# SmartBFT-Go/consensus

Hardware: NVIDIA H100
Metric: ECDSA-P256 verifies/sec at batch=64K (higher is better)
Workload: dtype u32 limbs (integer)

## Files before the change

### consensus_b200/csrc/hostsim.h

```cpp
#pragma once
#if defined(SBV_HOSTSIM) && !defined(__CUDACC__)
#include <stdint.h>
#include <string.h>

#include <condition_variable>
#include <map>
#include <mutex>

#define __device__
#define __host__
#define __global__
#define __forceinline__ inline
#define __noinline__
#define __restrict__
#define __shared__
#define __constant__ static const
#define __launch_bounds__(...)

struct hostsim_dim3 { unsigned x = 1, y = 1, z = 1; };
extern thread_local hostsim_dim3 threadIdx, blockIdx, blockDim, gridDim;
struct uint4 { uint32_t x, y, z, w; };
struct uint2 { uint32_t x, y; };
static inline uint4 make_uint4(uint32_t x, uint32_t y, uint32_t z, uint32_t w) { return uint4{x, y, z, w}; }

template <class T> static inline T __ldg(const T *p) { return *p; }
static inline uint32_t __byte_perm(uint32_t x, uint32_t y, uint32_t s) {
    const uint64_t v = ((uint64_t)y << 32) | x;
    uint32_t r = 0;
    for (int i = 0; i < 4; i++) {
        const uint32_t sel = (s >> (4 * i)) & 0xf;
        uint32_t byte = (uint32_t)(v >> (8 * (sel & 7))) & 0xff;
        if (sel & 8) byte = (byte & 0x80) ? 0xff : 0;
        r |= byte << (8 * i);
    }
    return r;
}
static inline uint32_t __funnelshift_r(uint32_t lo, uint32_t hi, uint32_t sh) {
    return (uint32_t)((((uint64_t)hi << 32) | lo) >> (sh & 31));
}
static inline uint32_t __funnelshift_l(uint32_t lo, uint32_t hi, uint32_t sh) {
    return (uint32_t)(((((uint64_t)hi << 32) | lo) << (sh & 31)) >> 32);
}
static inline int __ffs(int x) { return x ? __builtin_ctz((unsigned)x) + 1 : 0; }
static inline int __clz(int x) { return x ? __builtin_clz((unsigned)x) : 32; }
static inline int __popc(unsigned x) { return __builtin_popcount(x); }
static inline uint32_t __umulhi(uint32_t a, uint32_t b) { return (uint32_t)(((uint64_t)a * b) >> 32); }
static inline void __syncthreads() {}
static inline void __syncwarp(unsigned = 0xffffffffu) {}
static inline void __threadfence() {}
struct hostsim_warp {
    std::mutex m;
    std::condition_variable cv;
    struct Slot { unsigned arrived = 0, gen = 0; uint32_t in[32] = {}, out[32] = {}; };
    std::map<unsigned, Slot> slots;
};
extern thread_local hostsim_warp *hostsim_ctx;
static inline void hostsim_exchange(unsigned mask, uint32_t v, uint32_t (&all)[32]) {
    hostsim_warp *w = hostsim_ctx;
    std::unique_lock<std::mutex> lk(w->m);
    hostsim_warp::Slot &s = w->slots[mask];
    s.in[threadIdx.x & 31] = v;
    if (++s.arrived == (unsigned)__builtin_popcount(mask)) {
        memcpy(s.out, s.in, sizeof s.in);
        s.arrived = 0;
        s.gen++;
        w->cv.notify_all();
    } else {
        const unsigned g = s.gen;
        w->cv.wait(lk, [&] { return s.gen != g; });
    }
    memcpy(all, s.out, sizeof s.out);
}
static inline unsigned __ballot_sync(unsigned mask, int p) {
    if (!hostsim_ctx) return p ? 1u : 0u;
    uint32_t all[32];
    hostsim_exchange(mask, p ? 1u : 0u, all);
    unsigned r = 0;
    for (int i = 0; i < 32; i++) if (((mask >> i) & 1) && all[i]) r |= 1u << i;
    return r;
}
static inline unsigned __activemask() { return 1u; }
static inline unsigned __match_any_sync(unsigned mask, uint32_t v) {
    if (!hostsim_ctx) return 1u << (threadIdx.x & 31);
    uint32_t all[32];
    hostsim_exchange(mask, v, all);
    unsigned r = 0;
    for (int i = 0; i < 32; i++) if (((mask >> i) & 1) && all[i] == v) r |= 1u << i;
    return r;
}
template <class T> static inline T __shfl_sync(unsigned mask, T v, int src) {
    static_assert(sizeof(T) == 4, "32-bit shuffles only");
    if (!hostsim_ctx) return v;
    uint32_t u, all[32];
    memcpy(&u, &v, 4);
    hostsim_exchange(mask, u, all);
    T r;
    memcpy(&r, &all[src & 31], 4);
    return r;
}
template <class T> static inline T __shfl_down_sync(unsigned mask, T v, int delta) {
    if (!hostsim_ctx) return v;
    const int src = (int)(threadIdx.x & 31) + delta;
    const T r = __shfl_sync(mask, v, src > 31 ? (int)(threadIdx.x & 31) : src);
    return src > 31 ? v : r;
}
template <class T> static inline T atomicAdd(T *p, T v) { T o = *p; *p = o + v; return o; }
template <class T> static inline T atomicCAS(T *p, T cmp, T v) { T o = *p; if (o == cmp) *p = v; return o; }
template <class T> static inline T atomicMax(T *p, T v) { T o = *p; if (v > o) *p = v; return o; }
template <class T> static inline T atomicOr(T *p, T v) { T o = *p; *p = o | v; return o; }
typedef int cudaError_t;
typedef void *cudaStream_t;
#endif
```

### consensus_b200/csrc/inst_common.cuh

```cuda
#pragma once
#include "key_cache.cuh"
#include "keygroup.cuh"
#include "ops.h"

namespace sbv {

template <class C> struct Cfg;
template <> struct Cfg<P256> {
    static constexpr int COZ_MINB = 6, GPART_MINB = 6, KT_MINB = 6, COMB_MINB = 6;
    static constexpr bool KT_INL = true, COMB_INL = true;
};
template <> struct Cfg<P384> {
    static constexpr int COZ_MINB = 4, GPART_MINB = 3, KT_MINB = 4;
    static constexpr bool KT_INL = false;
};

template <class C>
cudaError_t op_gtable_init(uint32_t *gtab, cudaStream_t st) {
    const size_t entries = (size_t)C::GWINS << C::GW;
    k_gtable_init<C><<<(unsigned)((entries + 127) / 128), 128, 0, st>>>(gtab);
    return cudaGetLastError();
}

template <class C>
cudaError_t op_prep(uint32_t n, const uint8_t *r, const uint8_t *s, const uint8_t *dig, uint32_t dlen, uint32_t *uw, uint8_t *flags,
                    cudaStream_t st) {
    return launch_prep<C, 8>(n, r, s, dig, dlen, uw, flags, st);
}

template <class C>
cudaError_t op_group(uint32_t n, const uint8_t *qx, const uint8_t *qy, uint32_t seed, uint32_t hmask, uint32_t *htab, uint32_t *rep,
                     uint32_t *kcnt, uint32_t threshold, uint32_t max_keys, int32_t *keyid, uint32_t *keylist, uint32_t *counters,
                     cudaStream_t st) {
    const unsigned blocks = (n + 255) / 256;
    k_kg_insert<<<blocks, 256, 0, st>>>(n, KgXY<C>{qx, qy}, seed, hmask, htab, rep, kcnt);
    k_kg_assign<<<blocks, 256, 0, st>>>(n, rep, kcnt, threshold, max_keys, keyid, keylist, counters);
    return cudaGetLastError();
}

inline cudaError_t op_route(uint32_t n, const uint32_t *rep, const int32_t *keyid, int32_t *item_kid, uint32_t *klist, uint32_t *glist,
                            uint32_t *counters, cudaStream_t st) {
    k_kg_route<<<(n + 255) / 256, 256, 0, st>>>(n, rep, keyid, item_kid, klist, glist, counters);
    return cudaGetLastError();
}

template <class C>
cudaError_t op_gpart(uint32_t n, const uint32_t *uw, const uint32_t *gtab, uint32_t *gacc, cudaStream_t st) {
    constexpr int BLOCK = 64;
    k_gpart<C, BLOCK, Cfg<C>::GPART_MINB><<<(n + BLOCK - 1) / BLOCK, BLOCK, 0, st>>>(n, uw, reinterpret_cast<const uint4 *>(gtab), gacc);
    return cudaGetLastError();
}

template <class C>
cudaError_t op_coz(uint32_t n, const uint8_t *qx, const uint8_t *qy, const uint8_t *r, const uint32_t *uw, const uint8_t *flags,
                   const uint32_t *gtab, uint32_t *tscr, uint8_t *ok, const uint32_t *list, const uint32_t *count, cudaStream_t st) {
    constexpr int BLOCK = 64;
    const size_t smem = (size_t)7 * 2 * C::N * 4 * BLOCK;
    k_verify_coz<C, BLOCK, Cfg<C>::COZ_MINB><<<(n + BLOCK - 1) / BLOCK, BLOCK, smem, st>>>(
        n, qx, qy, r, uw, flags, reinterpret_cast<const uint4 *>(gtab), tscr, ok, list, count);
    return cudaGetLastError();
}

template <class C, int W>
cudaError_t op_kt_build(const uint32_t *nkeys_ptr, uint32_t cap, const uint32_t *keylist, const uint8_t *qx, const uint8_t *qy,
                        uint32_t *bases, uint32_t *hs, uint32_t *ztop, uint32_t *pref, uint32_t *ktab, uint8_t *keyflags, cudaStream_t st) {
    using KT = KeyTab<32 * C::N, W>;
    const unsigned kb = (cap + 63) / 64;
    const unsigned wb = (unsigned)(((size_t)cap * KT::NWIN + 63) / 64);
    k_kt_bases4<C, KT><<<(unsigned)(((size_t)cap * 4 + 127) / 128), 128, 0, st>>>(nkeys_ptr, cap, keylist, qx, qy, bases, keyflags);
    k_kt_fill<C, W><<<wb, 64, 0, st>>>(nkeys_ptr, cap, bases, keyflags, hs, ztop, ktab);
    k_kt_inv<C, KT><<<kb, 64, 0, st>>>(nkeys_ptr, cap, keyflags, ztop, pref);
    k_kt_final<C, KT><<<wb, 64, 0, st>>>(nkeys_ptr, cap, bases, keyflags, hs, ztop, ktab);
    return cudaGetLastError();
}

template <class C, int W>
cudaError_t op_kt_verify_grouped(uint32_t n, const int32_t *kidmap, const uint8_t *keyflags, const uint8_t *r, const uint32_t *uw, const uint8_t *flags,
                                 const uint32_t *gtab, const uint32_t *ktab, uint8_t *ok, const uint32_t *list, const uint32_t *count,
                                 const uint32_t *gacc, cudaStream_t st) {
    constexpr int BLOCK = 64;
    k_verify_kt<C, W, BLOCK, Cfg<C>::KT_MINB, false, Cfg<C>::KT_INL><<<(n + BLOCK - 1) / BLOCK, BLOCK, 0, st>>>(
        n, nullptr, kidmap, 0, keyflags, r, uw, flags, reinterpret_cast<const uint4 *>(gtab), reinterpret_cast<const uint4 *>(ktab), ok, list, count,
        gacc);
    return cudaGetLastError();
}

template <class C, int W>
cudaError_t op_kt_verify_registered(uint32_t n, const uint32_t *slot, const int32_t *slot2local, uint32_t n_slots, const uint8_t *keyflags,
                                    const uint8_t *r, const uint32_t *uw, const uint8_t *flags, const uint32_t *gtab, const uint32_t *ktab,
                                    uint8_t *ok, int warp, cudaStream_t st) {
    constexpr int BLOCK = 64;
    const uint4 *g4 = reinterpret_cast<const uint4 *>(gtab), *k4 = reinterpret_cast<const uint4 *>(ktab);
    if (warp)
        k_verify_kt_warp<C, W><<<(unsigned)(((size_t)n * 32 + 127) / 128), 128, 0, st>>>(n, slot, slot2local, n_slots, keyflags, r, uw, flags, g4, k4, ok);
    else
        k_verify_kt<C, W, BLOCK, Cfg<C>::KT_MINB, true, Cfg<C>::KT_INL><<<(n + BLOCK - 1) / BLOCK, BLOCK, 0, st>>>(
            n, slot, slot2local, n_slots, keyflags, r, uw, flags, g4, k4, ok, nullptr, nullptr, nullptr);
    return cudaGetLastError();
}

template <class C>
cudaError_t op_comb_build(const uint32_t *nkeys_ptr, uint32_t cap, const uint32_t *keylist, const uint8_t *qx, const uint8_t *qy,
                          uint32_t *bases, uint32_t *hs, uint32_t *ztop, uint32_t *pref, uint32_t *ktab, uint8_t *keyflags, cudaStream_t st) {
    using CT = CombTab<C>;
    const unsigned kb = (cap + 63) / 64;
    const unsigned cb = (unsigned)(((size_t)cap * CT::NCHAIN + 63) / 64);
    constexpr bool INL = Cfg<C>::COMB_INL;
    k_kt_bases2<C, CT, INL><<<(unsigned)(((size_t)cap * 2 + 127) / 128), 128, 0, st>>>(nkeys_ptr, cap, keylist, qx, qy, bases, keyflags);
    k_comb_affine<C><<<kb, 64, 0, st>>>(nkeys_ptr, cap, keyflags, bases, pref);
    k_comb_fill<C, INL><<<cb, 64, 0, st>>>(nkeys_ptr, cap, bases, keyflags, hs, ztop, ktab);
    k_kt_inv<C, CT><<<kb, 64, 0, st>>>(nkeys_ptr, cap, keyflags, ztop, pref);
    k_kt_final<C, CT, INL><<<cb, 64, 0, st>>>(nkeys_ptr, cap, bases, keyflags, hs, ztop, ktab);
    return cudaGetLastError();
}

template <class C>
cudaError_t op_comb_verify(uint32_t n, const int32_t *kidmap, const uint8_t *keyflags, const uint8_t *r, const uint32_t *uw, const uint8_t *flags,
                           const uint32_t * , const uint32_t *ktab, uint8_t *ok, const uint32_t *list,
                           const uint32_t *count, const uint32_t *gacc, cudaStream_t st) {
    constexpr int BLOCK = 64;
    k_verify_comb<C, BLOCK, Cfg<C>::COMB_MINB, Cfg<C>::COMB_INL><<<(n + BLOCK - 1) / BLOCK, BLOCK, 0, st>>>(
        n, kidmap, keyflags, r, uw, flags, reinterpret_cast<const uint4 *>(ktab), ok, list, count, gacc);
    return cudaGetLastError();
}

template <class C>
cudaError_t op_kc_lookup(const uint32_t *nkeys_ptr, uint32_t kcap, const uint32_t *keylist, const uint8_t *qx, const uint8_t *qy, KcMap c, uint32_t tw4,
                         int32_t *keyid, uint32_t *lk, uint8_t *keyflags, uint32_t *ktab, cudaStream_t st) {
    k_kc_lookup<<<(unsigned)(((size_t)kcap * 32 + 127) / 128), 128, 0, st>>>(nkeys_ptr, kcap, keylist, KcXY<C>{qx, qy}, c, tw4, keyid, lk, keyflags,
                                                                            reinterpret_cast<uint4 *>(ktab));
    return cudaGetLastError();
}

template <class C>
cudaError_t op_kc_insert(uint32_t kcap, const uint32_t *lk, const uint8_t *qx, const uint8_t *qy, KcMap c, uint32_t tw4, const uint8_t *keyflags,
                         const uint32_t *ktab, cudaStream_t st) {
    k_kc_insert<<<(unsigned)(((size_t)kcap * 32 + 127) / 128), 128, 0, st>>>(kcap, lk, KcXY<C>{qx, qy}, c, tw4, keyflags,
                                                                            reinterpret_cast<const uint4 *>(ktab));
    return cudaGetLastError();
}

template <class C, class KT>
constexpr KtGeom kt_geom() {
    using KS = KtSizes<C, KT>;
    return KtGeom{KS::bases_words(1), KS::hs_words(1), KS::ztop_words(1), KS::ktab_words(1)};
}

}
```

### consensus_b200/csrc/keygroup.cuh

```cuda
#pragma once
#include "kernels.cuh"

namespace sbv {

constexpr uint32_t KG_EMPTY = 0xffffffffu;

SBV_DEV uint32_t kg_mix(uint32_t h, uint32_t w) {
    h = (h ^ w) * 0x9E3779B1u;
    h ^= h >> 15;
    return h * 0x85EBCA77u;
}
template <class C>
SBV_DEV uint32_t kg_hash(const uint8_t *__restrict__ qx_be, const uint8_t *__restrict__ qy_be, uint32_t i, uint32_t seed) {
    const uint32_t *x = reinterpret_cast<const uint32_t *>(qx_be + (size_t)i * C::BYTES);
    const uint32_t *y = reinterpret_cast<const uint32_t *>(qy_be + (size_t)i * C::BYTES);
    uint32_t h = seed;
#pragma unroll
    for (int k = 0; k < C::N; k++) {
        h = kg_mix(h, __ldg(x + k));
        h = kg_mix(h, __ldg(y + k));
    }
    return h ^ (h >> 16);
}
template <class C>
SBV_DEV bool kg_same_key(const uint8_t *__restrict__ qx_be, const uint8_t *__restrict__ qy_be, uint32_t i, uint32_t j) {
    const uint32_t *xi = reinterpret_cast<const uint32_t *>(qx_be + (size_t)i * C::BYTES);
    const uint32_t *xj = reinterpret_cast<const uint32_t *>(qx_be + (size_t)j * C::BYTES);
    const uint32_t *yi = reinterpret_cast<const uint32_t *>(qy_be + (size_t)i * C::BYTES);
    const uint32_t *yj = reinterpret_cast<const uint32_t *>(qy_be + (size_t)j * C::BYTES);
    uint32_t diff = 0;
#pragma unroll
    for (int k = 0; k < C::N; k++) diff |= (__ldg(xi + k) ^ __ldg(xj + k)) | (__ldg(yi + k) ^ __ldg(yj + k));
    return diff == 0;
}

template <class C>
struct KgXY {
    const uint8_t *qx_be, *qy_be;
    SBV_DEV uint32_t hash(uint32_t i, uint32_t seed) const { return kg_hash<C>(qx_be, qy_be, i, seed); }
    SBV_DEV bool same(uint32_t i, uint32_t j) const { return kg_same_key<C>(qx_be, qy_be, i, j); }
};
struct KgKey32 {
    const uint8_t *pub;
    SBV_DEV uint32_t hash(uint32_t i, uint32_t seed) const {
        const uint32_t *x = reinterpret_cast<const uint32_t *>(pub + (size_t)i * 32);
        uint32_t h = seed;
#pragma unroll
        for (int k = 0; k < 8; k += 2) {
            h = (h ^ __ldg(x + k)) * 0x9E3779B1u;
            h = (h ^ __ldg(x + k + 1)) * 0x85EBCA77u;
            h ^= h >> 15;
        }
        return h;
    }
    SBV_DEV bool same(uint32_t i, uint32_t j) const {
        const uint32_t *xi = reinterpret_cast<const uint32_t *>(pub + (size_t)i * 32);
        const uint32_t *xj = reinterpret_cast<const uint32_t *>(pub + (size_t)j * 32);
        uint32_t diff = 0;
#pragma unroll
        for (int k = 0; k < 8; k++) diff |= __ldg(xi + k) ^ __ldg(xj + k);
        return diff == 0;
    }
};

template <class KV>
__global__ void __launch_bounds__(256) k_kg_insert(uint32_t n, KV key, uint32_t seed, uint32_t hmask, uint32_t *__restrict__ htab,
                                                   uint32_t *__restrict__ rep, uint32_t *__restrict__ kcnt) {
    const uint32_t i = blockIdx.x * blockDim.x + threadIdx.x;
    if (i >= n) return;
    uint32_t h = key.hash(i, seed) & hmask;
    uint32_t r;
    for (;;) {
        uint32_t cur = htab[h];
        if (cur == KG_EMPTY) {
            cur = atomicCAS(htab + h, KG_EMPTY, i);
            if (cur == KG_EMPTY) { r = i; break; }
        }
        if (key.same(i, cur)) { r = cur; break; }
        h = (h + 1) & hmask;
    }
    rep[i] = r;
#if defined(__CUDA_ARCH__)
    const uint32_t peers = __match_any_sync(__activemask(), r);
    if ((threadIdx.x & 31) == (uint32_t)(__ffs((int)peers) - 1)) atomicAdd(kcnt + r, (uint32_t)__popc(peers));
#else
    atomicAdd(kcnt + r, 1u);
#endif
}

static __global__ void __launch_bounds__(256) k_kg_assign(uint32_t n, const uint32_t *__restrict__ rep, const uint32_t *__restrict__ kcnt,
                                                   uint32_t threshold, uint32_t max_keys, int32_t *__restrict__ keyid,
                                                   uint32_t *__restrict__ keylist, uint32_t *__restrict__ counters) {
    const uint32_t i = blockIdx.x * blockDim.x + threadIdx.x;
    if (i >= n) return;
    int32_t id = -1;
    if (rep[i] == i && kcnt[i] >= threshold) {
        const uint32_t k = atomicAdd(counters + 0, 1u);
        if (k < max_keys) { id = (int32_t)k; keylist[k] = i; }
    }
    keyid[i] = id;
}

static __global__ void __launch_bounds__(256) k_kg_route(uint32_t n, const uint32_t *__restrict__ rep, const int32_t *__restrict__ keyid,
                                                  int32_t *__restrict__ item_kid, uint32_t *__restrict__ klist, uint32_t *__restrict__ glist,
                                                  uint32_t *__restrict__ counters) {
    const uint32_t i = blockIdx.x * blockDim.x + threadIdx.x;
    const bool live = i < n;
    const int32_t kid = live ? keyid[rep[i]] : -1;
    if (live) item_kid[i] = kid;
#if defined(__CUDA_ARCH__)
    const uint32_t lane = threadIdx.x & 31;
    const uint32_t mk = __ballot_sync(0xffffffffu, live && kid >= 0), mg = __ballot_sync(0xffffffffu, live && kid < 0);
    uint32_t bk = 0, bg = 0;
    if (lane == 0) {
        if (mk) bk = atomicAdd(counters + 1, (uint32_t)__popc(mk));
        if (mg) bg = atomicAdd(counters + 2, (uint32_t)__popc(mg));
    }
    bk = __shfl_sync(0xffffffffu, bk, 0);
    bg = __shfl_sync(0xffffffffu, bg, 0);
    const uint32_t below = (1u << lane) - 1u;
    if (live && kid >= 0) klist[bk + __popc(mk & below)] = i;
    if (live && kid < 0) glist[bg + __popc(mg & below)] = i;
#else
    if (live && kid >= 0) klist[atomicAdd(counters + 1, 1u)] = i;
    if (live && kid < 0) glist[atomicAdd(counters + 2, 1u)] = i;
#endif
}


template <class C, class KT>
__global__ void __launch_bounds__(64) k_kt_bases(const uint32_t *__restrict__ nkeys_ptr, uint32_t cap, const uint32_t *__restrict__ keylist,
                                                 const uint8_t *__restrict__ qx_be, const uint8_t *__restrict__ qy_be,
                                                 uint32_t *__restrict__ bases, uint8_t *__restrict__ keyflags) {
    constexpr int N = C::N;
    const uint32_t k = blockIdx.x * blockDim.x + threadIdx.x;
    uint32_t nkeys = __ldg(nkeys_ptr);
    if (nkeys > cap) nkeys = cap;
    if (k >= nkeys) return;
    const uint32_t item = keylist ? keylist[k] : k;
    Jac<C> B;
    const bool good = load_key<C>(B.X, B.Y, qx_be, qy_be, item);
    keyflags[k] = good ? 1 : 0;
    if (!good) return;
    C::get_one(B.Z);
#pragma unroll 1
    for (int win = 0; win < KT::NBASE; win++) {
        if (win) {
#pragma unroll 1
            for (int d = 0; d < KT::STEP; d++) pt_double<C>(B);
        }
        uint32_t *o = bases + (size_t)win * 3 * N * cap + k;
#pragma unroll
        for (int i = 0; i < N; i++) { o[(size_t)i * cap] = B.X[i]; o[(size_t)(N + i) * cap] = B.Y[i]; o[(size_t)(2 * N + i) * cap] = B.Z[i]; }
    }
}

template <class C, class KT>
__global__ void __launch_bounds__(128) k_kt_bases4(const uint32_t *__restrict__ nkeys_ptr, uint32_t cap, const uint32_t *__restrict__ keylist,
                                                   const uint8_t *__restrict__ qx_be, const uint8_t *__restrict__ qy_be,
                                                   uint32_t *__restrict__ bases, uint8_t *__restrict__ keyflags) {
    constexpr int N = C::N;
    const uint32_t gt = blockIdx.x * blockDim.x + threadIdx.x;
    const uint32_t k = gt >> 2, role = gt & 3;
    uint32_t nkeys = __ldg(nkeys_ptr);
    if (nkeys > cap) nkeys = cap;
    if (k >= nkeys) return;
    const unsigned qbase = (threadIdx.x & 31) & ~3u, qmask = 0xFu << qbase;
    const uint32_t item = keylist ? keylist[k] : k;
    uint32_t X[N], Y[N], Z[N];
    const bool good = load_key<C>(X, Y, qx_be, qy_be, item);
    if (role == 0) keyflags[k] = good ? 1 : 0;
    if (!good) return;
    C::get_one(Z);
    auto bcast = [&](uint32_t (&v)[N], unsigned src) {
#pragma unroll
        for (int i = 0; i < N; i++) v[i] = __shfl_sync(qmask, v[i], qbase + src);
    };
#pragma unroll 1
    for (int win = 0; win < KT::NBASE; win++) {
        if (win) {
#pragma unroll 1
            for (int d = 0; d < KT::STEP; d++) {
                uint32_t s[N], a[N], b[N], r1[N], r2[N], r3[N], r4[N], t1[N], t2[N];
                C::fadd(s, Y, Y);
                mp_select<N>(a, role == 1 || role == 2, s, Z);
                mp_select<N>(b, role == 1, s, Z);
                C::fmul(r1, a, b);
                uint32_t bb[N];
                mp_copy<N>(bb, r1);
                bcast(bb, 1);
                C::fsub(t1, X, r1);
                C::fadd(t2, X, r1);
                mp_select<N>(a, role == 0, t1, X);
                mp_select<N>(a, role == 2, bb, a);
                mp_select<N>(b, role == 0, t2, bb);
                C::fmul(r2, a, b);
                uint32_t alpha[N], half[N], beta4[N];
                C::fadd(t1, r2, r2);
                C::fadd(alpha, t1, r2);
                C::fhalf(half, r2);
                C::fmul(r3, alpha, alpha);
                mp_copy<N>(beta4, r2);
                bcast(beta4, 1);
                bcast(half, 2);
                uint32_t x3[N], y3[N];
                C::fadd(t1, beta4, beta4);
                C::fsub(x3, r3, t1);
                C::fsub(t2, beta4, x3);
                C::fmul(r4, alpha, t2);
                C::fsub(y3, r4, half);
                mp_copy<N>(X, x3); bcast(X, 0);
                mp_copy<N>(Y, y3); bcast(Y, 0);
                mp_copy<N>(Z, r1); bcast(Z, 2);
            }
        }
        if (role == 0) {
            uint32_t *o = bases + (size_t)win * 3 * N * cap + k;
#pragma unroll
            for (int i = 0; i < N; i++) { o[(size_t)i * cap] = X[i]; o[(size_t)(N + i) * cap] = Y[i]; o[(size_t)(2 * N + i) * cap] = Z[i]; }
        }
    }
}

template <class C, class KT, bool INL>
__global__ void __launch_bounds__(128) k_kt_bases2(const uint32_t *__restrict__ nkeys_ptr, uint32_t cap, const uint32_t *__restrict__ keylist,
                                                   const uint8_t *__restrict__ qx_be, const uint8_t *__restrict__ qy_be,
                                                   uint32_t *__restrict__ bases, uint8_t *__restrict__ keyflags) {
    using A = typename PickArith<C, INL>::type;
    constexpr int N = C::N;
    const uint32_t gt = blockIdx.x * blockDim.x + threadIdx.x;
    const uint32_t k = gt >> 1, role = gt & 1;
    uint32_t nkeys = __ldg(nkeys_ptr);
    if (nkeys > cap) nkeys = cap;
    if (k >= nkeys) return;
    const unsigned pbase = (threadIdx.x & 31) & ~1u, pmask = 3u << pbase, other = pbase + (role ^ 1);
    const uint32_t item = keylist ? keylist[k] : k;
    uint32_t X[N], Y[N], Z[N];
    const bool good = load_key<C>(X, Y, qx_be, qy_be, item);
    if (role == 0) keyflags[k] = good ? 1 : 0;
    if (!good) return;
    C::get_one(Z);
    auto xchg = [&](uint32_t (&v)[N]) {
#pragma unroll
        for (int i = 0; i < N; i++) v[i] = __shfl_sync(pmask, v[i], other);
    };
#pragma unroll 1
    for (int win = 0; win < KT::NBASE; win++) {
        if (win) {
#pragma unroll 1
            for (int d = 0; d < KT::STEP; d++) {
                uint32_t s[N], a[N], b[N], r1[N], r2[N], r3[N], r4[N], t1[N], t2[N];
                C::fadd(s, Y, Y);
                mp_select<N>(a, role == 1, s, Z);
                A::fsqr(r1, a);
                C::fsub(t1, X, r1);
                C::fadd(t2, X, r1);
                mp_select<N>(a, role == 1, X, t1);
                mp_select<N>(b, role == 1, r1, t2);
                A::fmul(r2, a, b);
                uint32_t beta4[N], alpha[N];
                mp_copy<N>(beta4, r2);
                xchg(beta4);
                C::fadd(t1, r2, r2);
                C::fadd(alpha, t1, r2);
                mp_select<N>(a, role == 1, r1, alpha);
                A::fsqr(r3, a);
                uint32_t x3[N], c8[N];
                C::fadd(t1, beta4, beta4);
                C::fsub(t2, r3, t1);
                C::fhalf(t1, r3);
                mp_select<N>(x3, role == 1, t1, t2);
                xchg(x3);
                mp_select<N>(c8, role == 1, t1, x3);
                mp_select<N>(x3, role == 1, x3, t2);
                C::fsub(t1, beta4, x3);
                mp_select<N>(a, role == 1, s, alpha);
                mp_select<N>(b, role == 1, Z, t1);
                A::fmul(r4, a, b);
                C::fsub(t2, r4, c8);
                mp_select<N>(t1, role == 1, r4, t2);
                xchg(t1);
                mp_copy<N>(X, x3);
                mp_select<N>(Y, role == 1, t1, t2);
                mp_select<N>(Z, role == 1, r4, t1);
            }
        }
        if (role == 0) {
            uint32_t *o = bases + (size_t)win * 3 * N * cap + k;
#pragma unroll
            for (int i = 0; i < N; i++) { o[(size_t)i * cap] = X[i]; o[(size_t)(N + i) * cap] = Y[i]; o[(size_t)(2 * N + i) * cap] = Z[i]; }
        }
    }
}

template <int N>
SBV_DEV void st_entry(uint32_t *o, const uint32_t (&x)[N], const uint32_t (&y)[N]) {
    uint4 *v = reinterpret_cast<uint4 *>(o);
#pragma unroll
    for (int i = 0; i < N / 4; i++) {
        uint4 a, b;
        a.x = x[4 * i]; a.y = x[4 * i + 1]; a.z = x[4 * i + 2]; a.w = x[4 * i + 3];
        b.x = y[4 * i]; b.y = y[4 * i + 1]; b.z = y[4 * i + 2]; b.w = y[4 * i + 3];
        v[i] = a;
        v[N / 4 + i] = b;
    }
}
template <int N>
SBV_DEV void ld_entry(const uint32_t *o, uint32_t (&x)[N], uint32_t (&y)[N]) {
    const uint4 *v = reinterpret_cast<const uint4 *>(o);
#pragma unroll
    for (int i = 0; i < N / 4; i++) {
        const uint4 a = v[i], b = v[N / 4 + i];
        x[4 * i] = a.x; x[4 * i + 1] = a.y; x[4 * i + 2] = a.z; x[4 * i + 3] = a.w;
        y[4 * i] = b.x; y[4 * i + 1] = b.y; y[4 * i + 2] = b.z; y[4 * i + 3] = b.w;
    }
}

template <class C>
SBV_DEV void zaddu(uint32_t (&X1)[C::N], uint32_t (&Y1)[C::N], const uint32_t (&X2)[C::N], const uint32_t (&Y2)[C::N],
                   uint32_t (&X3)[C::N], uint32_t (&Y3)[C::N], uint32_t (&h)[C::N]) {
    constexpr int N = C::N;
    uint32_t c[N], w1[N], w2[N], dy[N], d[N], a1[N], t[N];
    C::fsub(h, X1, X2);
    C::fsqr(c, h);
    C::fmul(w1, X1, c);
    C::fmul(w2, X2, c);
    C::fsub(dy, Y1, Y2);
    C::fsqr(d, dy);
    C::fsub(t, w1, w2);
    C::fmul(a1, Y1, t);
    C::fsub(X3, d, w1);
    C::fsub(X3, X3, w2);
    C::fsub(t, w1, X3);
    C::fmul(Y3, dy, t);
    C::fsub(Y3, Y3, a1);
    mp_copy<N>(X1, w1);
    mp_copy<N>(Y1, a1);
}

template <class C, int W>
__global__ void __launch_bounds__(64) k_kt_fill(const uint32_t *__restrict__ nkeys_ptr, uint32_t cap, const uint32_t *__restrict__ bases,
                                                const uint8_t *__restrict__ keyflags, uint32_t *__restrict__ hs,
                                                uint32_t *__restrict__ ztop, uint32_t *__restrict__ ktab) {
    constexpr int N = C::N;
    using KT = KeyTab<32 * N, W>;
    const uint32_t t = blockIdx.x * blockDim.x + threadIdx.x;
    uint32_t nkeys = __ldg(nkeys_ptr);
    if (nkeys > cap) nkeys = cap;
    if (t >= nkeys * KT::NWIN) return;
    const uint32_t k = t % nkeys, win = t / nkeys;
    if (!keyflags[k]) return;
    uint32_t bx[N], by[N], bz[N];
    {
        const uint32_t *o = bases + (size_t)win * 3 * N * cap + k;
#pragma unroll
        for (int i = 0; i < N; i++) { bx[i] = o[(size_t)i * cap]; by[i] = o[(size_t)(N + i) * cap]; bz[i] = o[(size_t)(2 * N + i) * cap]; }
    }
    uint32_t *out = ktab + ((size_t)k * KT::NWIN + win) * KT::ENT * 2 * N;
#pragma unroll
    for (int i = 0; i < N; i++) { out[i] = bx[i]; out[N + i] = by[i]; }
    Jac<C> P;
    mp_copy<N>(P.X, bx); mp_copy<N>(P.Y, by); mp_copy<N>(P.Z, bz);
    uint32_t h[N], h2[N], h3[N];
    C::fadd(h, by, by);
    pt_double<C>(P);
    C::fsqr(h2, h);
    C::fmul(h3, h2, h);
    C::fmul(bx, bx, h2);
    C::fmul(by, by, h3);
    uint32_t zacc[N];
    mp_copy<N>(zacc, P.Z);
    {
        uint32_t *hp = hs + ((size_t)win * (KT::ENT - 1) + 0) * N * cap + k;
#pragma unroll
        for (int i = 0; i < N; i++) { out[2 * N + i] = P.X[i]; out[3 * N + i] = P.Y[i]; hp[(size_t)i * cap] = h[i]; }
    }
    uint32_t px[N], py[N];
    mp_copy<N>(px, P.X); mp_copy<N>(py, P.Y);
#pragma unroll 1
    for (int e = 3; e <= KT::ENT; e++) {
        uint32_t x3[N], y3[N];
        zaddu<C>(bx, by, px, py, x3, y3, h);
        C::fmul(zacc, zacc, h);
        mp_copy<N>(px, x3); mp_copy<N>(py, y3);
        uint32_t *hp = hs + ((size_t)win * (KT::ENT - 1) + (e - 2)) * N * cap + k;
        uint32_t *oe = out + (size_t)(e - 1) * 2 * N;
#pragma unroll
        for (int i = 0; i < N; i++) { oe[i] = px[i]; oe[N + i] = py[i]; hp[(size_t)i * cap] = h[i]; }
    }
    uint32_t *zp = ztop + (size_t)win * N * cap + k;
#pragma unroll
    for (int i = 0; i < N; i++) zp[(size_t)i * cap] = zacc[i];
}

template <class C, class KT>
__global__ void __launch_bounds__(64) k_kt_inv(const uint32_t *__restrict__ nkeys_ptr, uint32_t cap, const uint8_t *__restrict__ keyflags,
                                               uint32_t *__restrict__ ztop, uint32_t *__restrict__ pref) {
    constexpr int N = C::N;
    const uint32_t k = blockIdx.x * blockDim.x + threadIdx.x;
    uint32_t nkeys = __ldg(nkeys_ptr);
    if (nkeys > cap) nkeys = cap;
    if (k >= nkeys || !keyflags[k]) return;
    uint32_t run[N];
    C::get_one(run);
#pragma unroll 1
    for (int win = 0; win < KT::NCHAIN; win++) {
        uint32_t z[N];
        const uint32_t *zp = ztop + (size_t)win * N * cap + k;
        uint32_t *pp = pref + (size_t)win * N * cap + k;
#pragma unroll
        for (int i = 0; i < N; i++) { z[i] = zp[(size_t)i * cap]; pp[(size_t)i * cap] = run[i]; }
        C::fmul(run, run, z);
    }
    uint32_t inv[N];
    p_inv<C>(inv, run);
#pragma unroll 1
    for (int win = KT::NCHAIN - 1; win >= 0; win--) {
        uint32_t z[N], pv[N], zi[N];
        uint32_t *zp = ztop + (size_t)win * N * cap + k;
        const uint32_t *pp = pref + (size_t)win * N * cap + k;
#pragma unroll
        for (int i = 0; i < N; i++) { z[i] = zp[(size_t)i * cap]; pv[i] = pp[(size_t)i * cap]; }
        C::fmul(zi, inv, pv);
        C::fmul(inv, inv, z);
#pragma unroll
        for (int i = 0; i < N; i++) zp[(size_t)i * cap] = zi[i];
    }
}

template <class C, class KT, bool INL = false>
__global__ void __launch_bounds__(64) k_kt_final(const uint32_t *__restrict__ nkeys_ptr, uint32_t cap, const uint32_t *__restrict__ bases,
                                                 const uint8_t *__restrict__ keyflags, const uint32_t *__restrict__ hs,
                                                 const uint32_t *__restrict__ ztop, uint32_t *__restrict__ ktab) {
    using A = typename PickArith<C, INL>::type;
    constexpr int N = C::N;
    const uint32_t t = blockIdx.x * blockDim.x + threadIdx.x;
    uint32_t nkeys = __ldg(nkeys_ptr);
    if (nkeys > cap) nkeys = cap;
    if (t >= nkeys * KT::NCHAIN) return;
    const uint32_t k = t % nkeys, win = t / nkeys;
    if (!keyflags[k]) return;
    uint32_t zi[N];
    {
        const uint32_t *zp = ztop + (size_t)win * N * cap + k;
#pragma unroll
        for (int i = 0; i < N; i++) zi[i] = zp[(size_t)i * cap];
    }
    uint32_t *out = ktab + ((size_t)k * KT::NCHAIN + win) * KT::ENT * 2 * N;
    uint32_t x[N], y[N], h[N];
    {
        ld_entry<N>(out + (size_t)(KT::ENT - 1) * 2 * N, x, y);
    }
#pragma unroll 1
    for (int e = KT::ENT; e >= 1; e--) {
        uint32_t nx[N], ny[N], nh[N];
        if (e >= 2) {
            const uint32_t *hp = hs + ((size_t)win * (KT::ENT - 1) + (e - 2)) * N * cap + k;
            ld_entry<N>(out + (size_t)(e - 2) * 2 * N, nx, ny);
#pragma unroll
            for (int i = 0; i < N; i++) nh[i] = hp[(size_t)i * cap];
        }
        uint32_t z2[N], z3[N];
        A::fsqr(z2, zi);
        A::fmul(z3, z2, zi);
        A::fmul(x, x, z2);
        A::fmul(y, y, z3);
        st_entry<N>(out + (size_t)(e - 1) * 2 * N, x, y);
        if (e >= 2) {
            mp_copy<N>(h, nh);
            A::fmul(zi, zi, h);
            mp_copy<N>(x, nx); mp_copy<N>(y, ny);
        }
    }
    (void)bases;
}


template <class C>
__global__ void __launch_bounds__(64) k_comb_affine(const uint32_t *__restrict__ nkeys_ptr, uint32_t cap, const uint8_t *__restrict__ keyflags,
                                                    uint32_t *__restrict__ bases, uint32_t *__restrict__ pref) {
    constexpr int N = C::N;
    using CT = CombTab<C>;
    const uint32_t k = blockIdx.x * blockDim.x + threadIdx.x;
    uint32_t nkeys = __ldg(nkeys_ptr);
    if (nkeys > cap) nkeys = cap;
    if (k >= nkeys || !keyflags[k]) return;
    uint32_t run[N];
    C::get_one(run);
#pragma unroll 1
    for (int c = 0; c < CT::NBASE; c++) {
        uint32_t z[N];
        const uint32_t *zp = bases + ((size_t)c * 3 + 2) * N * cap + k;
        uint32_t *pp = pref + (size_t)c * N * cap + k;
#pragma unroll
        for (int i = 0; i < N; i++) { z[i] = zp[(size_t)i * cap]; pp[(size_t)i * cap] = run[i]; }
        C::fmul(run, run, z);
    }
    uint32_t inv[N];
    p_inv<C>(inv, run);
#pragma unroll 1
    for (int c = CT::NBASE - 1; c >= 0; c--) {
        uint32_t *o = bases + (size_t)c * 3 * N * cap + k;
        const uint32_t *pp = pref + (size_t)c * N * cap + k;
        uint32_t x[N], y[N], z[N], pv[N], zi[N], z2[N], z3[N];
#pragma unroll
        for (int i = 0; i < N; i++) { x[i] = o[(size_t)i * cap]; y[i] = o[(size_t)(N + i) * cap]; z[i] = o[(size_t)(2 * N + i) * cap]; pv[i] = pp[(size_t)i * cap]; }
        C::fmul(zi, inv, pv);
        C::fmul(inv, inv, z);
        C::fsqr(z2, zi);
        C::fmul(z3, z2, zi);
        C::fmul(x, x, z2);
        C::fmul(y, y, z3);
#pragma unroll
        for (int i = 0; i < N; i++) { o[(size_t)i * cap] = x[i]; o[(size_t)(N + i) * cap] = y[i]; }
    }
}

template <class C, bool INL>
__global__ void __launch_bounds__(64) k_comb_fill(const uint32_t *__restrict__ nkeys_ptr, uint32_t cap, const uint32_t *__restrict__ bases,
                                                  const uint8_t *__restrict__ keyflags, uint32_t *__restrict__ hs,
                                                  uint32_t *__restrict__ ztop, uint32_t *__restrict__ ktab) {
    using A = typename PickArith<C, INL>::type;
    constexpr int N = C::N;
    using CT = CombTab<C>;
    const uint32_t t = blockIdx.x * blockDim.x + threadIdx.x;
    uint32_t nkeys = __ldg(nkeys_ptr);
    if (nkeys > cap) nkeys = cap;
    if (t >= nkeys * CT::NCHAIN) return;
    const uint32_t k = t % nkeys, ch = t / nkeys;
    if (!keyflags[k]) return;
    const int b = (int)(ch >> 4), hi = (int)(ch & 15);
    auto base = [&](int c, uint32_t (&x)[N], uint32_t (&y)[N]) {
        const uint32_t *o = bases + (size_t)c * 3 * N * cap + k;
#pragma unroll
        for (int i = 0; i < N; i++) { x[i] = o[(size_t)i * cap]; y[i] = o[(size_t)(N + i) * cap]; }
    };
    uint32_t *out = ktab + ((size_t)k * CT::NCHAIN + ch) * CT::ENT * 2 * N;
    auto store = [&](int slot, const uint32_t (&x)[N], const uint32_t (&y)[N], const uint32_t (&h)[N]) {
        st_entry<N>(out + (size_t)slot * 2 * N, x, y);
        if (slot) {
            uint32_t *hp = hs + ((size_t)ch * (CT::ENT - 1) + (slot - 1)) * N * cap + k;
#pragma unroll
            for (int i = 0; i < N; i++) hp[(size_t)i * cap] = h[i];
        }
    };
    Jac<A> P;
    uint32_t x[N], y[N], h[N], zero[N];
#pragma unroll
    for (int i = 0; i < N; i++) zero[i] = 0;
    C::get_one(P.Z);
    C::get_one(h);
    if (hi == 0) store(0, zero, zero, h);
    const int nhigh = __popc(hi);
    int rest = hi;
#pragma unroll 1
    for (int st = 0; st < nhigh + CT::ENT - 1; st++) {
        const int kk = st - nhigh + 1;
        int tooth;
        bool sub = false;
        if (kk <= 0) {
            tooth = 4 + __ffs(rest) - 1;
            rest &= rest - 1;
        } else {
            tooth = __ffs(kk) - 1;
            sub = !(((kk ^ (kk >> 1)) >> tooth) & 1);
        }
        base(CT::TEETH * b + tooth, x, y);
        if (sub) C::fsub(y, zero, y);
        if (st == 0) { mp_copy<N>(P.X, x); mp_copy<N>(P.Y, y); }
        else pt_madd_table<A>(P, x, y, h);
        if (kk >= 0) store(kk, P.X, P.Y, h);
    }
    uint32_t *zp = ztop + (size_t)ch * N * cap + k;
#pragma unroll
    for (int i = 0; i < N; i++) zp[(size_t)i * cap] = P.Z[i];
}

template <class C, class KT_>
struct KtSizes {
    using KT = KT_;
    static constexpr size_t bases_words(size_t cap) { return (size_t)KT::NBASE * 3 * C::N * cap; }
    static constexpr size_t hs_words(size_t cap) { return (size_t)KT::NCHAIN * (KT::ENT - 1) * C::N * cap; }
    static constexpr size_t ztop_words(size_t cap) { return (size_t)KT::NCHAIN * C::N * cap; }
    static constexpr size_t ktab_words(size_t cap) { return KT::POINTS * 2 * C::N * cap; }
};

}
```

Measured before the change: 71.84 million.

## Warp-per-key comb table build with shared-memory bases and key-major scratch layout

Replaces the per-thread comb fill and final kernels with warp-cooperative versions, one warp per key and one lane per chain. Each key's bases are staged in shared memory, the Jacobian and h intermediates are stored in a key-major uint4 layout, and output rows are transposed through shared memory so table writes are coalesced. The inversion kernel gains a pluggable z-layout so it matches the new scratch layout. This only touches per-key table precomputation, so batch verify throughput may barely change, and it adds shared memory use and warp syncs.

After: 76.75 million, median of 6. 6.8% higher.

```diff
diff --git a/consensus_b200/csrc/hostsim.h b/consensus_b200/csrc/hostsim.h
--- a/consensus_b200/csrc/hostsim.h
+++ b/consensus_b200/csrc/hostsim.h
@@ -46,7 +46,6 @@
 static inline int __popc(unsigned x) { return __builtin_popcount(x); }
 static inline uint32_t __umulhi(uint32_t a, uint32_t b) { return (uint32_t)(((uint64_t)a * b) >> 32); }
 static inline void __syncthreads() {}
-static inline void __syncwarp(unsigned = 0xffffffffu) {}
 static inline void __threadfence() {}
 struct hostsim_warp {
     std::mutex m;
@@ -70,6 +69,11 @@
         w->cv.wait(lk, [&] { return s.gen != g; });
     }
     memcpy(all, s.out, sizeof s.out);
+}
+static inline void __syncwarp(unsigned mask = 0xffffffffu) {
+    if (!hostsim_ctx) return;
+    uint32_t all[32];
+    hostsim_exchange(mask, 0, all);
 }
 static inline unsigned __ballot_sync(unsigned mask, int p) {
     if (!hostsim_ctx) return p ? 1u : 0u;
diff --git a/consensus_b200/csrc/inst_common.cuh b/consensus_b200/csrc/inst_common.cuh
--- a/consensus_b200/csrc/inst_common.cuh
+++ b/consensus_b200/csrc/inst_common.cuh
@@ -104,13 +104,15 @@
                           uint32_t *bases, uint32_t *hs, uint32_t *ztop, uint32_t *pref, uint32_t *ktab, uint8_t *keyflags, cudaStream_t st) {
     using CT = CombTab<C>;
     const unsigned kb = (cap + 63) / 64;
-    const unsigned cb = (unsigned)(((size_t)cap * CT::NCHAIN + 63) / 64);
+    const unsigned wb = (unsigned)(((size_t)cap * 32 + 63) / 64);
     constexpr bool INL = Cfg<C>::COMB_INL;
+    constexpr size_t fill_smem = (size_t)2 * CT::NBASE * 2 * C::N * 4;
+    constexpr size_t final_smem = (size_t)2 * 32 * (CT::ENT / 2 * 2 * C::N / 4 + 1) * 16;
     k_kt_bases2<C, CT, INL><<<(unsigned)(((size_t)cap * 2 + 127) / 128), 128, 0, st>>>(nkeys_ptr, cap, keylist, qx, qy, bases, keyflags);
     k_comb_affine<C><<<kb, 64, 0, st>>>(nkeys_ptr, cap, keyflags, bases, pref);
-    k_comb_fill<C, INL><<<cb, 64, 0, st>>>(nkeys_ptr, cap, bases, keyflags, hs, ztop, ktab);
-    k_kt_inv<C, CT><<<kb, 64, 0, st>>>(nkeys_ptr, cap, keyflags, ztop, pref);
-    k_kt_final<C, CT, INL><<<cb, 64, 0, st>>>(nkeys_ptr, cap, bases, keyflags, hs, ztop, ktab);
+    k_comb_fill_warp<C, INL><<<wb, 64, fill_smem, st>>>(nkeys_ptr, cap, bases, keyflags, hs, ztop);
+    k_kt_inv<C, CT, CombScr<C>><<<kb, 64, 0, st>>>(nkeys_ptr, cap, keyflags, ztop, pref);
+    k_comb_final<C, INL><<<wb, 64, final_smem, st>>>(nkeys_ptr, cap, keyflags, hs, ztop, ktab);
     return cudaGetLastError();
 }
 
diff --git a/consensus_b200/csrc/keygroup.cuh b/consensus_b200/csrc/keygroup.cuh
--- a/consensus_b200/csrc/keygroup.cuh
+++ b/consensus_b200/csrc/keygroup.cuh
@@ -393,7 +393,12 @@
     for (int i = 0; i < N; i++) zp[(size_t)i * cap] = zacc[i];
 }
 
-template <class C, class KT>
+template <int N>
+struct ZByChain {
+    SBV_DEV static size_t at(uint32_t k, int ch, int i, uint32_t cap) { return ((size_t)ch * N + i) * cap + k; }
+};
+
+template <class C, class KT, class ZL = ZByChain<C::N>>
 __global__ void __launch_bounds__(64) k_kt_inv(const uint32_t *__restrict__ nkeys_ptr, uint32_t cap, const uint8_t *__restrict__ keyflags,
                                                uint32_t *__restrict__ ztop, uint32_t *__restrict__ pref) {
     constexpr int N = C::N;
@@ -406,10 +411,12 @@
 #pragma unroll 1
     for (int win = 0; win < KT::NCHAIN; win++) {
         uint32_t z[N];
-        const uint32_t *zp = ztop + (size_t)win * N * cap + k;
-        uint32_t *pp = pref + (size_t)win * N * cap + k;
-#pragma unroll
-        for (int i = 0; i < N; i++) { z[i] = zp[(size_t)i * cap]; pp[(size_t)i * cap] = run[i]; }
+#pragma unroll
+        for (int i = 0; i < N; i++) {
+            const size_t a = ZL::at(k, win, i, cap);
+            z[i] = ztop[a];
+            pref[a] = run[i];
+        }
         C::fmul(run, run, z);
     }
     uint32_t inv[N];
@@ -417,14 +424,12 @@
 #pragma unroll 1
     for (int win = KT::NCHAIN - 1; win >= 0; win--) {
         uint32_t z[N], pv[N], zi[N];
-        uint32_t *zp = ztop + (size_t)win * N * cap + k;
-        const uint32_t *pp = pref + (size_t)win * N * cap + k;
-#pragma unroll
-        for (int i = 0; i < N; i++) { z[i] = zp[(size_t)i * cap]; pv[i] = pp[(size_t)i * cap]; }
+#pragma unroll
+        for (int i = 0; i < N; i++) { const size_t a = ZL::at(k, win, i, cap); z[i] = ztop[a]; pv[i] = pref[a]; }
         C::fmul(zi, inv, pv);
         C::fmul(inv, inv, z);
 #pragma unroll
-        for (int i = 0; i < N; i++) zp[(size_t)i * cap] = zi[i];
+        for (int i = 0; i < N; i++) ztop[ZL::at(k, win, i, cap)] = zi[i];
     }
 }
 
@@ -576,11 +581,152 @@
     for (int i = 0; i < N; i++) zp[(size_t)i * cap] = P.Z[i];
 }
 
+template <class C>
+struct CombScr {
+    using CT = CombTab<C>;
+    static constexpr int Q = C::N / 4;
+    static constexpr size_t KEY = (size_t)((CT::ENT - 1) * Q + CT::ENT * 2 * Q) * CT::NCHAIN;
+    SBV_DEV static size_t hs(uint32_t k, int slot, int w) { return k * KEY + ((size_t)(slot - 1) * Q + w) * CT::NCHAIN; }
+    SBV_DEV static size_t jac(uint32_t k, int slot, int w) { return k * KEY + ((size_t)(CT::ENT - 1) * Q + (size_t)slot * 2 * Q + w) * CT::NCHAIN; }
+    SBV_DEV static size_t z(uint32_t k, int w) { return ((size_t)k * Q + w) * CT::NCHAIN; }
+    SBV_DEV static size_t at(uint32_t k, int ch, int i, uint32_t) { return (z(k, i / 4) + ch) * 4 + (i & 3); }
+};
+
+template <int N>
+SBV_DEV uint4 quad(const uint32_t (&v)[N], int w) { return make_uint4(v[4 * w], v[4 * w + 1], v[4 * w + 2], v[4 * w + 3]); }
+template <int N>
+SBV_DEV void unquad(uint32_t (&v)[N], int w, const uint4 q) { v[4 * w] = q.x; v[4 * w + 1] = q.y; v[4 * w + 2] = q.z; v[4 * w + 3] = q.w; }
+
+template <class C, bool INL>
+__global__ void __launch_bounds__(64) k_comb_fill_warp(const uint32_t *__restrict__ nkeys_ptr, uint32_t cap, const uint32_t *__restrict__ bases,
+                                                       const uint8_t *__restrict__ keyflags, uint32_t *__restrict__ hs, uint32_t *__restrict__ ztop) {
+    using A = typename PickArith<C, INL>::type;
+    constexpr int N = C::N, Q = N / 4, HT = CombTab<C>::TEETH / 2;
+    using CT = CombTab<C>;
+    using S = CombScr<C>;
+    static_assert(CT::NCHAIN == 32 && CT::NBASE * 2 == 32, "a lane per chain; a lane per coordinate of a base");
+    const uint32_t k = (blockIdx.x * blockDim.x + threadIdx.x) >> 5, ch = threadIdx.x & 31;
+    uint32_t nkeys = __ldg(nkeys_ptr);
+    if (nkeys > cap) nkeys = cap;
+    if (k >= nkeys || !keyflags[k]) return;
+    extern __shared__ uint32_t tab[];
+    uint32_t *pb = tab + (threadIdx.x >> 5) * CT::NBASE * 2 * N;
+    {
+        const uint32_t *o = bases + ((size_t)(ch >> 1) * 3 + (ch & 1)) * N * cap + k;
+#pragma unroll
+        for (int i = 0; i < N; i++) pb[ch * N + i] = o[(size_t)i * cap];
+    }
+    __syncwarp();
+    uint4 *h4 = reinterpret_cast<uint4 *>(hs), *z4 = reinterpret_cast<uint4 *>(ztop);
+    auto store = [&](int slot, const uint32_t (&x)[N], const uint32_t (&y)[N], const uint32_t (&h)[N]) {
+#pragma unroll
+        for (int w = 0; w < Q; w++) { h4[S::jac(k, slot, w) + ch] = quad<N>(x, w); h4[S::jac(k, slot, Q + w) + ch] = quad<N>(y, w); }
+        if (slot) {
+#pragma unroll
+            for (int w = 0; w < Q; w++) h4[S::hs(k, slot, w) + ch] = quad<N>(h, w);
+        }
+    };
+    const int b = (int)(ch >> 4), hi = (int)(ch & 15), nhigh = __popc(hi);
+    Jac<A> P;
+    uint32_t x[N], y[N], h[N], zero[N];
+#pragma unroll
+    for (int i = 0; i < N; i++) zero[i] = 0;
+    C::get_one(P.Z);
+    C::get_one(h);
+    if (hi == 0) store(0, zero, zero, h);
+    int rest = hi;
+#pragma unroll 1
+    for (int s = 0; s < HT + CT::ENT - 1; s++) {
+        const int st = s - (HT - nhigh);
+        if (st < 0) continue;
+        const int kk = s - (HT - 1);
+        int tooth;
+        bool neg = false;
+        if (kk <= 0) {
+            tooth = HT + __ffs(rest) - 1;
+            rest &= rest - 1;
+        } else {
+            tooth = __ffs(kk) - 1;
+            neg = !(((kk ^ (kk >> 1)) >> tooth) & 1);
+        }
+        const uint32_t *pt = pb + (CT::TEETH * b + tooth) * 2 * N;
+#pragma unroll
+        for (int i = 0; i < N; i++) { x[i] = pt[i]; y[i] = pt[N + i]; }
+        if (neg) C::fsub(y, zero, y);
+        if (st == 0) { mp_copy<N>(P.X, x); mp_copy<N>(P.Y, y); }
+        else pt_madd_table<A>(P, x, y, h);
+        if (kk >= 0) store(kk, P.X, P.Y, h);
+    }
+#pragma unroll
+    for (int w = 0; w < Q; w++) z4[S::z(k, w) + ch] = quad<N>(P.Z, w);
+}
+
+template <class C, bool INL>
+__global__ void __launch_bounds__(64) k_comb_final(const uint32_t *__restrict__ nkeys_ptr, uint32_t cap, const uint8_t *__restrict__ keyflags,
+                                                   const uint32_t *__restrict__ hs, const uint32_t *__restrict__ ztop, uint32_t *__restrict__ ktab) {
+    using A = typename PickArith<C, INL>::type;
+    constexpr int N = C::N, Q = N / 4;
+    using CT = CombTab<C>;
+    using S = CombScr<C>;
+    constexpr int HALF = CT::ENT / 2, ROW = HALF * 2 * Q + 1;
+    static_assert(CT::NCHAIN == 32 && HALF * 2 * Q == 32, "a lane per chain; a half chain is one 16-byte word per lane");
+    const uint32_t k = (blockIdx.x * blockDim.x + threadIdx.x) >> 5, ch = threadIdx.x & 31;
+    uint32_t nkeys = __ldg(nkeys_ptr);
+    if (nkeys > cap) nkeys = cap;
+    if (k >= nkeys || !keyflags[k]) return;
+    extern __shared__ uint32_t tab[];
+    uint4 *stage = reinterpret_cast<uint4 *>(tab) + (threadIdx.x >> 5) * 32 * ROW;
+    const uint4 *h4 = reinterpret_cast<const uint4 *>(hs), *z4 = reinterpret_cast<const uint4 *>(ztop);
+    uint4 *out = reinterpret_cast<uint4 *>(ktab) + (size_t)k * CT::POINTS * 2 * Q;
+    uint32_t zi[N];
+#pragma unroll
+    for (int w = 0; w < Q; w++) unquad<N>(zi, w, z4[S::z(k, w) + ch]);
+    auto load = [&](int slot, uint32_t (&x)[N], uint32_t (&y)[N]) {
+#pragma unroll
+        for (int w = 0; w < Q; w++) { unquad<N>(x, w, h4[S::jac(k, slot, w) + ch]); unquad<N>(y, w, h4[S::jac(k, slot, Q + w) + ch]); }
+    };
+    uint32_t x[N], y[N];
+    load(CT::ENT - 1, x, y);
+#pragma unroll 1
+    for (int e = CT::ENT; e >= 1; e--) {
+        uint32_t nx[N], ny[N], nh[N];
+        if (e >= 2) {
+            load(e - 2, nx, ny);
+#pragma unroll
+            for (int w = 0; w < Q; w++) unquad<N>(nh, w, h4[S::hs(k, e - 1, w) + ch]);
+        }
+        uint32_t z2[N], z3[N];
+        A::fsqr(z2, zi);
+        A::fmul(z3, z2, zi);
+        A::fmul(x, x, z2);
+        A::fmul(y, y, z3);
+        uint4 *row = stage + ch * ROW + ((e - 1) % HALF) * 2 * Q;
+#pragma unroll
+        for (int w = 0; w < Q; w++) { row[w] = quad<N>(x, w); row[Q + w] = quad<N>(y, w); }
+        if ((e - 1) % HALF == 0) {
+            __syncwarp();
+            uint4 *o = out + (size_t)(e - 1) * 2 * Q + ch;
+#pragma unroll 4
+            for (int j = 0; j < CT::NCHAIN; j++) o[(size_t)j * CT::ENT * 2 * Q] = stage[j * ROW + ch];
+            __syncwarp();
+        }
+        if (e >= 2) {
+            A::fmul(zi, zi, nh);
+            mp_copy<N>(x, nx); mp_copy<N>(y, ny);
+        }
+    }
+}
+
+template <class KT> struct IsComb { static constexpr bool value = false; };
+template <class C> struct IsComb<CombTab<C>> { static constexpr bool value = true; };
+
 template <class C, class KT_>
 struct KtSizes {
     using KT = KT_;
     static constexpr size_t bases_words(size_t cap) { return (size_t)KT::NBASE * 3 * C::N * cap; }
-    static constexpr size_t hs_words(size_t cap) { return (size_t)KT::NCHAIN * (KT::ENT - 1) * C::N * cap; }
+    static constexpr size_t hs_words(size_t cap) {
+        return IsComb<KT>::value ? CombScr<C>::KEY * 4 * cap : (size_t)KT::NCHAIN * (KT::ENT - 1) * C::N * cap;
+    }
     static constexpr size_t ztop_words(size_t cap) { return (size_t)KT::NCHAIN * C::N * cap; }
     static constexpr size_t ktab_words(size_t cap) { return KT::POINTS * 2 * C::N * cap; }
 };
```
